# dflemin3/approxposterior

Hardware: AMD Instinct MI355X
Metric: GP-predict+acquisition candidates/sec (N_train, D fixed) (higher is better)
Workload: dtype f64

## Files before the change

### approxposterior_amd/_lib.py

```python
import ctypes
import os

_HERE = os.path.dirname(os.path.abspath(__file__))
LIB_PATH = os.path.join(_HERE, "csrc", "libapgp.so")
ABI_VERSION = 8
MAX_DIM = 32
MAX_FANTASY = 32
MAX_DRAWS = 32
MAX_FEATURES = 65536
MAX_REFS = 4096
INTEGRATED_MAX_DIM = 16

UTIL_AGP, UTIL_BAPE, UTIL_JONES, UTIL_NONE = 0, 1, 2, 3
UTIL_NEG_MEAN = 4
NM_MAX_RESTARTS = 4096
NM_MAX_FEV = 1 << 20
NM_STEPS = {1: "reflect", 2: "expand", 3: "reflect_exp", 4: "contract_out", 5: "contract_in",
            6: "shrink_out", 7: "shrink_in", 8: "maxfev"}
PRUNE_ROWS_SPLIT, PRUNE_ROWS_SIGNED = 0, 1
GMM_EM, GMM_SCORE, GMM_KMEANS = 0, 1, 2
GMM_MAX_COMP = 16
IMP_BLOCK = 256
IMP_MAX_BLOCKS = 2048

# ... 66 lines not shown
    "apgp_trsv_ex": (ctypes.c_int, [_P, _I64, _I64, _P, _F64, ctypes.c_int, _P, _P, ctypes.c_int, _P]),
    "apgp_trsv_mode": (ctypes.c_int, [ctypes.c_int]),
    "apgp_append_diag": (ctypes.c_int, [_P, _P, _F64, _P, _I64, _P]),
    "apgp_winv_apply_work_len": (_I64, [_I64]),
    "apgp_winv_apply": (ctypes.c_int, [_P, _I64, _I64, _P, _F64, ctypes.c_int, _P, _P, _P, _P]),
    "apgp_trtri_pack": (ctypes.c_int, [_P, _I64, _I64, _P, _P, _P, _P]),
    "apgp_pack_train": (ctypes.c_int, [_P, _P, _I64, _KP, _P, _P]),
    "apgp_acquire": (ctypes.c_int, [_P, _I64, _I64, _P, _P, _I64, _KP, _F64, _I32,
                                    ctypes.POINTER(_F64), ctypes.POINTER(_F64), _P,
                                    _F64, _F64, _P, _P, _P, _P, _P, _P]),
    "apgp_packed_lsolve_len": (_I64, [_I64]),
    "apgp_pack_lsolve": (ctypes.c_int, [_P, _I64, _I64, _P, _P]),
    "apgp_acquire_solve": (ctypes.c_int, [_P, _I64, _I64, _P, _P, _I64, _KP, _F64, _I32,
                                          ctypes.POINTER(_F64), ctypes.POINTER(_F64), _P,
                                          _F64, _F64, _P, _P, _P, _P, _P, _P]),
    "apgp_set_sweep_prune": (ctypes.c_int, [ctypes.c_int]),
    "apgp_get_sweep_prune": (ctypes.c_int, []),
    "apgp_set_seed_rowsplit": (ctypes.c_int, [ctypes.c_int]),
    "apgp_get_seed_rowsplit": (ctypes.c_int, []),
    "apgp_set_seed_park": (ctypes.c_int, [ctypes.c_int]),
    "apgp_get_seed_park": (ctypes.c_int, []),
    "apgp_set_prune_pipe": (ctypes.c_int, [ctypes.c_int]),
    "apgp_get_prune_pipe": (ctypes.c_int, []),
    "apgp_set_seed_first": (ctypes.c_int, [ctypes.c_int]),
    "apgp_get_seed_first": (ctypes.c_int, []),
    "apgp_set_seed_parts": (ctypes.c_int, [ctypes.c_int]),
    "apgp_get_seed_parts": (ctypes.c_int, []),
    "apgp_sweep_prune_counts_offset": (_I64, [_I64, _I64]),
    "apgp_sweep_prune_select": (ctypes.c_int, [_P, _I64, _P, _P, _F64, _P, _P]),
    "apgp_prune_bounds": (ctypes.c_int, [_P, _I64, _P, _I64, _KP, _F64, _I32, ctypes.POINTER(_F64), ctypes.POINTER(_F64),
                                         _P, _F64, _F64, ctypes.c_int, _P, _P]),
    "apgp_sweep_prune_seeds": (ctypes.c_int, [_P, _I64, _P, _P, _P]),
    "apgp_prune_rows_len": (_I64, [_I64, _I32]),
    "apgp_pack_prune_rows": (ctypes.c_int, [_P, _I64, _KP, _P, _P]),
    "apgp_acquire_rows": (ctypes.c_int, [_P, _I64, _I64, _P, _P, _I64, _KP, _F64, _I32,
                                         ctypes.POINTER(_F64), ctypes.POINTER(_F64), _P,
                                         _F64, _F64, _P, _P, _P, _P, _P, _P, _P]),
    "apgp_acquire_solve_rows": (ctypes.c_int, [_P, _I64, _I64, _P, _P, _I64, _KP, _F64, _I32,
                                               ctypes.POINTER(_F64), ctypes.POINTER(_F64), _P,
                                               _F64, _F64, _P, _P, _P, _P, _P, _P, _P]),
    "apgp_prune_bounds_rows": (ctypes.c_int, [_P, _I64, _P, _I64, _KP, _F64, _I32, ctypes.POINTER(_F64),
                                              ctypes.POINTER(_F64), _P, _F64, _F64, ctypes.c_int, _P, _P, _P]),
    "apgp_prune_srows_len": (_I64, [_I64, _I32]),
    "apgp_pack_prune_srows": (ctypes.c_int, [_P, _I64, _KP, _P, _P]),
    "apgp_acquire_rows2": (ctypes.c_int, [_P, _I64, _I64, _P, _P, _I64, _KP, _F64, _I32,
                                          ctypes.POINTER(_F64), ctypes.POINTER(_F64), _P,
# ... 108 lines not shown
```

### approxposterior_amd/csrc/sweep.hip

```cpp
#include "apgp_common.h"
#include "mma16.h"
#include "scratch.h"
#include "util_value.h"
#include <mutex>
#include <stdlib.h>
#include <string.h>

#define SW_ROWS APGP_ROW_BLOCK
#define SW_KC APGP_K_CHUNK
#define SW_TILE (SW_ROWS * SW_KC)
#define SW_CAND 64
#define SW_GRID 256
#define SW_BCH 1024
typedef unsigned int u32x4 __attribute__((ext_vector_type(4)));
#ifndef SW_KAUX
#define SW_KAUX 0
#endif

struct SweepArgs {
    const double* T;
    const double* linv;
    const double* xs;
    const unsigned char* mask;
    double* mu;
// ... 52 lines not shown
#define S2_NP (S2_ROWS / 32)
#define S2_STATIC_DIAG_NRB 8

#define S2_HQ_PRE (4 * 256)
#define S2_HQ_ACC (56 * 256)
#define S2_SPLIT_MAX 184
#define S2_PRUNE_WORDS 24
__host__ __device__ inline long long s2_fold_off(int nrb, long long ncb) {
    return (2ll * S2_SPLIT_MAX * SW_CAND * nrb + 3 * ncb + S2_PRUNE_WORDS + 1) & ~1ll;
}
__host__ __device__ inline double* s2_fold_item(double* sp_q, int nrb, long long ncb, long long pos, int jb) {
    return sp_q + s2_fold_off(nrb, ncb) + (pos * nrb + jb) * (S2_HQ_PRE + S2_HQ_ACC);
}
#define S2_HALF_COST 7
#define S2_WHOLE_COST 10
#define S2P_HALF_GEN 340
#define S2P_HALF_PARK 116
#define S2P_WHOLE_GEN 197
#define S2P_WHOLE_PARK 232
#define S2P_PAIR2_GEN 187
#define S2P_PAIR2_PARK 98
#define S2P_PAIR1_GEN 161
#define S2P_PAIR1_PARK 81
#define S2P_WAVE2 2000
#define S2W_WORD(j0, lg, p0, p1) ((2 + (j0)) | ((lg) << 8) | ((p0) << 12) | ((p1) << 20))
#define S2W_J0(sp) (((sp) & 0xff) - 2)
#define S2W_LG(sp) (((sp) >> 8) & 3)
#define S2W_P0(sp) (((sp) >> 12) & 31)
#define S2W_P1(sp) (((sp) >> 20) & 31)
#define S2W_SEED (1 << 28)
__host__ __device__ inline int s2_nkc_of(int jb, int n) {
    const int v = S2_CPB * (jb + 1), lim = (n + SW_KC - 1) / SW_KC;
    return v < lim ? v : lim;
}
__host__ __device__ inline int s2_nparts(int jb, int j0, int n, int lg) {
    if (jb < j0 || lg == 0) return 1;
    const int per = S2_ROWS >> lg, c = (n - S2_ROWS * jb + per - 1) / per;
    return c > (1 << lg) ? (1 << lg) : (c < 1 ? 1 : c);
}
__host__ __device__ inline int s2_nitems(int nrb, int j0, int n, int lg) {
    int c = 0;
    for (int jb = 0; jb < nrb; ++jb) c += s2_nparts(jb, j0, n, lg);
    return c;
}
__host__ __device__ inline int s2_part_cost(int lg) { return lg == 0 ? S2_WHOLE_COST : lg == 1 ? S2_HALF_COST : lg == 2 ? 5 : 4; }
__host__ __device__ inline void s2_row_item(int idx, int nrb, int j0, int n, int lg, int& jb, int& h) {
    int hj = nrb - 1, hh = hj >= 0 ? s2_nparts(hj, j0, n, lg) - 1 : 0, wj = (j0 < nrb ? j0 : nrb) - 1;
    const int pc = s2_part_cost(lg);
    for (int i = 0;; ++i) {
        if (hj >= j0 && (wj < 0 || pc * s2_nkc_of(hj, n) >= S2_WHOLE_COST * s2_nkc_of(wj, n))) {
            const int np = s2_nparts(hj, j0, n, lg);
            if (i == idx) { jb = hj; h = np > 1 ? hh : -1; return; }
            if (hh > 0) --hh; else { --hj; hh = hj >= 0 ? s2_nparts(hj, j0, n, lg) - 1 : 0; }
// ... 1 lines not shown
            if (i == idx || wj < 0) { jb = wj < 0 ? 0 : wj; h = -1; return; }
            --wj;
        }
    }
}
__device__ __forceinline__ double s2_q_gather(const double (&qr)[4], int lane) {
    double qs = qr[0];
#pragma unroll
    for (int r = 1; r < 4; ++r) qs += __shfl(qr[r], (lane & 48) | ((lane - 4 * r) & 15));
    qs += __shfl_xor(qs, 16);
    qs += __shfl_xor(qs, 32);
    return qs;
}
__device__ __forceinline__ bool s2_wave_skip(const SweepArgs& a, int nrb, int p0, long long pos) {
    if (p0 == 0) return false;
    const double* bmin = a.sp_q + 2ll * S2_SPLIT_MAX * SW_CAND * nrb;
    double tau = INFINITY;
    for (int i = 0; i < p0; ++i) tau = fmin(tau, a.part_u[a.blk_list[i]]);
    return !(bmin[a.blk_list[pos]] <= tau);
}

static constexpr bool s2_structured_feeder(int dpad, bool solve) { return dpad == 32 ? false : (solve ? dpad == 2 : dpad != 8); }

template <int DPAD, bool LIN, int MODE, bool LIST = false, bool RHALF = false>
__global__ __launch_bounds__(S2_THREADS, 1) void sweep2_kernel(SweepArgs a) {
    static_assert(!RHALF || (MODE == 0 && LIST), "row-half items: inverse form, list launches");
    constexpr bool SOLVE = MODE != 0;
    constexpr bool SPARK = RHALF && !LIN;
    constexpr bool STATIC_DIAG = MODE == 2;
    constexpr int XS = DPAD + 2;
    constexpr int NKK = SW_KC / 4;
    constexpr int NP = S2_NP;
    constexpr int XCHUNK16 = SW_KC * XS / 2;
    constexpr bool SF = s2_structured_feeder(DPAD, SOLVE);
    constexpr int XSTRIDE = SF ? (SW_KC * XS * 8 + 1023) / 1024 * 128 : SW_KC * XS;
    extern __shared__ __attribute__((aligned(16))) double smem[];
    double* Aring = smem;
    double* Bbuf = Aring + 3 * S2_TILE;
    double* Xbuf = Bbuf + 2 * 4 * 256;
    double* Etab = Xbuf + (SF ? 3 : 2) * XSTRIDE;
    double* Shq = Etab + APGP_EXP_TAB_N;
    double* red_u = Shq + SW_CAND;
    long long* red_i = (long long*)(red_u + 4);
    double* Cst = red_u + 8;
    const int t = threadIdx.x, lane = t & 63, w = t >> 6;
    const int cl = lane & 15, kq = lane >> 4;
    long long lst_end = 0;
    [[maybe_unused]] int wv_n = 0;
    if constexpr (LIST) {
// ... 27 lines not shown
    const int kc_lim = (a.n + SW_KC - 1) / SW_KC;
    const int nrb2 = (a.n + S2_ROWS - 1) / S2_ROWS;
    auto nkc_of = [&](int jb) { const int v = S2_CPB * (jb + 1); return v < kc_lim ? v : kc_lim; };
    auto tile_off = [&](int jb, int kc) {
        const int ib = jb >> 1;
        const unsigned tile = (unsigned)((SW_ROWS / SW_KC) * ib * (ib + 1) / 2 + kc);
        return tile * (unsigned)(SW_TILE * 8) + (unsigned)((jb & 1) * S2_TILE * 8);
    };
    int jb_lo = 0, jb_hi = nrb2;
    int rh = -1;
    long long blk0 = S2_BLK_BEGIN + blockIdx.x, blk_step = gridDim.x;
    if (a.split) {
        const int nsplit = RHALF ? wv_n : (int)(S2_BLK_END - S2_BLK_BEGIN);
        blk0 = S2_BLK_BEGIN + (int)blockIdx.x % nsplit;
        if constexpr (RHALF) {
            blk0 += S2W_P0(a.split);
            s2_row_item((int)blockIdx.x / nsplit, nrb2, S2W_J0(a.split), a.n, S2W_LG(a.split), jb_lo, rh);
        } else jb_lo = nrb2 - 1 - (int)blockIdx.x / nsplit;
        jb_hi = jb_lo + 1;
        blk_step = S2_BLK_END;
    }
    const int rpp = RHALF ? S2_NP >> S2W_LG(a.split) : S2_NP;
    const int rsh = rh > 0 ? rh * rpp : 0;
    auto successor = [&](int& jb, int& kc, long long& blk) {
        ++kc;
        if (kc >= nkc_of(jb)) { ++jb; kc = 0; }
        if (jb >= jb_hi) { jb = jb_lo; blk += blk_step; }
    };

    if (w < 4) {
        int lr[4];
#pragma unroll
        for (int r = 0; r < 4; ++r) lr[r] = (lane & 48) | ((lane + 4 * r) & 15);
        f64x2 av[2][2][2];
        auto load_a = [&](f64x2 (&dst)[2][2], int slot, int p) {
            const f64x2* A2 = (const f64x2*)(Aring + slot * S2_TILE) + lane;
#pragma unroll
            for (int h = 0; h < 2; ++h)
#pragma unroll
                for (int kp = 0; kp < 2; ++kp) dst[h][kp] = A2[((p * 2 + h) * 2 + kp) * 64];
        };
        __syncthreads();
        __syncthreads();
        __syncthreads();
        int slot = 0, bpar = 0;
        double brot[4][NKK];
        auto load_b = [&](int buf, int half) {
            const f64x2* Bw = (const f64x2*)(Bbuf + buf * 1024 + w * 256) + half * 64;
#pragma unroll
            for (int r = 0; r < 4; ++r) {
                const f64x2 bv = Bw[lr[r]];
                brot[r][2 * half] = bv.x; brot[r][2 * half + 1] = bv.y;
            }
        };
        load_a(av[0], 0, 0);
        load_b(0, 0);
        const __amdgpu_buffer_rsrc_t rs_kv = __builtin_amdgcn_make_buffer_rsrc(
            (void*)(a.kcache + (long long)blockIdx.x * a.ncache * SW_BCH), 0, (int)a.kslot_bytes, 0x00020000);
        for (long long blk = blk0; blk < S2_BLK_END; blk += blk_step) {
            double qtot = 0.0;
            for (int jb = jb_lo; jb < jb_hi; ++jb) {
                const int nkc = nkc_of(jb);
                const int ndiag0 = S2_CPB * jb;
                double qmic = 0.0;
                double acc[2 * NP][4];
#pragma unroll
                for (int s_ = 0; s_ < 2 * NP; ++s_)
#pragma unroll
                    for (int r = 0; r < 4; ++r) acc[s_][r] = 0.0;
                int kc = 0;
                auto do_tile_n = [&](auto pred_tag, auto npa_tag) {
                    constexpr bool PRED = decltype(pred_tag)::value;
                    constexpr int NPA = decltype(npa_tag)::value;
                    const int nslot = slot == 2 ? 0 : slot + 1;
                    auto mfma_pair = [&](int pr, int kk) {
#pragma unroll
                        for (int r = 0; r < 4; ++r) {
                            acc[2 * pr][r] = __builtin_amdgcn_mfma_f64_4x4x4f64(
                                av[pr & 1][0][kk >> 1][kk & 1], brot[r][kk], acc[2 * pr][r], 0, 0, 0);
                            acc[2 * pr + 1][r] = __builtin_amdgcn_mfma_f64_4x4x4f64(
                                av[pr & 1][1][kk >> 1][kk & 1], brot[r][kk], acc[2 * pr + 1][r], 0, 0, 0);
                        }
                    };
                    int p0 = (kc - ndiag0) >> 1;
                    if constexpr (RHALF) p0 -= rsh;
                    if (p0 < 0) p0 = 0;
                    int p1 = (a.n - S2_ROWS * jb + 31) >> 5;
                    if constexpr (RHALF) {
                        p1 -= rsh;
                        if (rh >= 0 && p1 > rpp) p1 = rpp;
                    }
                    if (p1 > NP) p1 = NP;
#pragma unroll
                    for (int pr = 0; pr < NPA; ++pr) {
                        const bool act = !PRED || (pr >= p0 && pr < p1);
                        if (act) mfma_pair(pr, 0);
                        __builtin_amdgcn_sched_barrier(0);
                        if (pr == NPA / 2) {
                            if constexpr (SOLVE) asm volatile("s_waitcnt vmcnt(0)" ::: "memory");
                            __syncthreads();
                        }
                        if (pr + 1 < NPA) {
                            if (pr == 0) load_b(bpar, 1);
                            load_a(av[(pr + 1) & 1], slot, pr + 1);
                            if (act) {
                                mfma_pair(pr, 1);
                                mfma_pair(pr, 2);
                                mfma_pair(pr, 3);
                            }
#if S2_SPREAD > 0
                            if (!PRED) {
#pragma unroll
                                for (int q_ = 0; q_ < (pr == 0 ? 8 : 4); ++q_) {
                                    __builtin_amdgcn_sched_group_barrier(0x100, 1, 0);
                                    __builtin_amdgcn_sched_group_barrier(0x008, S2_SPREAD, 0);
                                }
                            }
#endif
                        } else {
                            load_a(av[0], nslot, 0);
                            if (act) mfma_pair(pr, 1);
                            __builtin_amdgcn_sched_barrier(0);
                            load_b(bpar ^ 1, 0);
                            if (act) {
                                mfma_pair(pr, 2);
                                mfma_pair(pr, 3);
                            }
#if S2_SPREAD > 0
                            if (!PRED) {
#pragma unroll
                                for (int q_ = 0; q_ < 4; ++q_) {
                                    __builtin_amdgcn_sched_group_barrier(0x100, 1, 0);
                                    __builtin_amdgcn_sched_group_barrier(0x008, S2_SPREAD, 0);
                                }
                            }
#endif
                        }
                        __builtin_amdgcn_sched_barrier(0);
                    }
                    slot = nslot;
                    bpar ^= 1;
                };
                auto do_tile = [&](auto pred_tag) { do_tile_n(pred_tag, std::integral_constant<int, NP>{}); };
                if constexpr (RHALF) {
                    const int nhalf4 = (rh >= 0 && rpp == 4) ? ndiag0 : 0;
                    for (; kc < nhalf4; ++kc) do_tile_n(std::false_type{}, std::integral_constant<int, 4>{});
// ... 301 lines not shown
        const bool inb = blk < a.blk_end && crow < a.m;
        bool adm = inb, has_nan = false;
        double ktl = (LIN && a.lin_order == 0) ? (double)a.ndim : 0.0;
#pragma unroll
        for (int d = 0; d < DPAD; ++d) {
            double v = 0.0;
            if (inb && d < a.ndim) {
                v = a.T[crow * a.ndim + d];
                if (a.has_box && !(v >= Cst[APGP_MAX_DIM + d] && v <= Cst[2 * APGP_MAX_DIM + d])) adm = false;
                if (v != v) has_nan = true;
            }
            tt[d] = v * Cst[d];
            if (LIN && a.lin_order > 0) {
                const double p = v * v;
                double q = p;
                for (int e = 1; e < a.lin_order; ++e) q *= p;
                ktl += q;
            }
        }
        if (inb && a.mask && a.mask[crow] == 0) adm = false;
        fl_cur = ((adm && !has_nan) ? 1 : 0) | (has_nan ? 2 : 0) | (inb ? 4 : 0);
        ktt_cur = LIN ? fma(a.lin_coef, ktl, a.amp) : a.amp;
    };
    auto produce_b = [&](int jb, int kc, int bb, int xb) {
        double bfv[NKK];
        {
            const double* Xb = Xbuf + xb * XSTRIDE;
            double s2[NKK], s3[NKK], al[NKK], lsum[NKK];
#pragma unroll
            for (int kk = 0; kk < NKK; ++kk) {
                s2[kk] = 0.0; s3[kk] = 0.0;
                lsum[kk] = (LIN && a.lin_order == 0) ? (double)a.ndim : 0.0;
                al[kk] = Xb[(kk * 4 + kq) * XS + DPAD];
            }
#pragma unroll
            for (int d = 0; d < DPAD; d += 2)
#pragma unroll
                for (int kk = 0; kk < NKK; ++kk) {
                    const f64x2 xa = *(const f64x2*)(Xb + (kk * 4 + kq) * XS + d);
                    const double df0 = tt[d] - xa.x, df1 = tt[d + 1] - xa.y;
                    s2[kk] = fma(df0, df0, s2[kk]);
                    s3[kk] = fma(df1, df1, s3[kk]);
                    if (LIN && a.lin_order > 0) {
                        const double p0_ = tt[d] * xa.x * Cst[3 * APGP_MAX_DIM + d], p1_ = tt[d + 1] * xa.y * Cst[3 * APGP_MAX_DIM + d + 1];
                        double q0 = p0_, q1 = p1_;
                        for (int e = 1; e < a.lin_order; ++e) { q0 *= p0_; q1 *= p1_; }
                        lsum[kk] += q0 + q1;
// ... 5 lines not shown
            apgp_exp4(ex, bfv, Etab);
#pragma unroll
            for (int kk = 0; kk < NKK; ++kk) bfv[kk] = LIN ? fma(a.lin_coef, lsum[kk], bfv[kk] * a.amp) : bfv[kk] * a.amp;
            if (kc >= S2_CPB * jb) {
#pragma unroll
                for (int kk = 0; kk < NKK; ++kk) mu_cur = fma(bfv[kk], al[kk], mu_cur);
                if (kc == nkc_of(jb) - 1) {
                    double m = mu_cur;
                    m += __shfl_xor(m, 16);
                    m += __shfl_xor(m, 32);
                    mu_tot += m;
                    mu_cur = 0.0;
                }
                if (!SOLVE && !SPARK && park && jb + 1 < nrb2) {
                    const unsigned soff = (unsigned)kc * (unsigned)(SW_BCH * 8);
                    f64x2 q0, q1;
                    q0.x = bfv[0]; q0.y = bfv[1]; q1.x = bfv[2]; q1.y = bfv[3];
                    __builtin_amdgcn_raw_buffer_store_b128(__builtin_bit_cast(u32x4, q0), rs_k, hoff, soff, SW_KAUX);
                    __builtin_amdgcn_raw_buffer_store_b128(__builtin_bit_cast(u32x4, q1), rs_k, hoff, soff + 256 * 16, SW_KAUX);
                }
            }
            f64x2 o0, o1;
            o0.x = bfv[0]; o0.y = bfv[1]; o1.x = bfv[2]; o1.y = bfv[3];
            if (bb == 0) { f64x2* Bw = (f64x2*)(Bbuf + hw * 256); Bw[lane] = o0; Bw[64 + lane] = o1; }
            else { f64x2* Bw = (f64x2*)(Bbuf + 1024 + hw * 256); Bw[lane] = o0; Bw[64 + lane] = o1; }
        }
    };
    auto epilogue = [&]() {
        __syncthreads();
        if (a.split) {
            if (kq == 0) {
                const long long e = ((LIST ? blk0 : blk_fin - a.blk_begin) * SW_CAND + hw * 16 + cl) * nrb2 + jb_lo;
                if (!RHALF || rh < 0) a.sp_q[e] = Shq[hw * 16 + cl];
                if (!RHALF || rh <= 0) a.sp_mu[e] = mu_fin;
            }
            __syncthreads();
            return;
        }
        double bu = INFINITY;
        long long bi = -1;
        const long long crow = blk_fin * SW_CAND + hw * 16 + cl;
        if (kq == 0 && (fl_fin & 4)) {
            double mu = mu_fin + a.mean;
            double var = ktt_fin - Shq[hw * 16 + cl];
            if (fl_fin & 2) { mu = NAN; var = NAN; }
            if (a.mu) a.mu[crow] = mu;
            if (a.var) a.var[crow] = var;
            if (a.kind != APGP_UTIL_NONE) {
                const double uu = (fl_fin & 1) ? util_value(a.kind, mu, var, a.zeta, a.ybest) : INFINITY;
                if (a.u) a.u[crow] = uu;
                best_merge(bu, bi, uu, a.idx_offset + crow);
            }
        }
        for (int o = 8; o > 0; o >>= 1) {
            double ou = __shfl_xor(bu, o);
            long long oi = __shfl_xor(bi, o);
            best_merge(bu, bi, ou, oi);
        }
        if (lane == 0) { red_u[hw] = bu; red_i[hw] = bi; }
        __syncthreads();
        if (ht == 0 && a.kind != APGP_UTIL_NONE) {
            for (int i = 1; i < 4; ++i) best_merge(bu, bi, red_u[i], red_i[i]);
            a.part_u[blk_fin] = bu;
            a.part_i[blk_fin] = bi;
        }
    };

    if constexpr (SF) {
        const int hw_s = __builtin_amdgcn_readfirstlane(hw);
        typedef __attribute__((address_space(3))) void lds_void;
        auto dma_tile = [&](int slot, int jb, int kc) {
            double* dst = Aring + slot * S2_TILE + hw_s * 128;
            const unsigned toffs = tile_off(jb, kc);
            if constexpr (RHALF) {
                if (rh >= 0) {
#pragma unroll
                    for (int q = 0; q < 4; ++q)
                        if (q < rpp)
                            __builtin_amdgcn_raw_ptr_buffer_load_lds(rs_w, (lds_void*)(dst + q * 512), 16, (unsigned)lane * 16u,
                                                                     toffs + (unsigned)((q + rsh) * 4096) + (unsigned)hw_s * 1024u, 0, 0);
                    return;
                }
            }
#pragma unroll
            for (int q = 0; q < 8; ++q)
                __builtin_amdgcn_raw_ptr_buffer_load_lds(rs_w, (lds_void*)(dst + q * 512), 16, (unsigned)lane * 16u,
                                                         toffs + (unsigned)(q * 4096) + (unsigned)hw_s * 1024u, 0, 0);
        };
        auto dma_parked = [&](int par, int c) {
            double* dst = Bbuf + par * 1024 + hw_s * 256;
// ... 297 lines not shown
static inline long long s2_ncache(int64_t n) { return (long long)S2_CPB * (s2_nrb(n) - 1); }

template <int DPAD>
static constexpr size_t s2_lds_bytes() {
    return (3 * S2_TILE + 2 * 4 * 256 + 3 * ((SW_KC * (DPAD + 2) * 8 + 1023) / 1024 * 128) + APGP_EXP_TAB_N + SW_CAND + 8 +
            4 * APGP_MAX_DIM) * sizeof(double);
}

template <int DPAD>
static int s2_prepare_device() {
    static ApgpLdsOnce once;
    int dev = 0;
    if (hipGetDevice(&dev) != hipSuccess || dev < 0 || dev >= 64) {
        apgp_set_error("apgp_acquire: hipGetDevice failed");
        return -2;
    }
    return apgp_raise_lds(once, "apgp_acquire", dev, (int)s2_lds_bytes<DPAD>(),
                          {(const void*)sweep2_kernel<DPAD, false, 0>, (const void*)sweep2_kernel<DPAD, true, 0>,
                           (const void*)sweep2_kernel<DPAD, false, 1>, (const void*)sweep2_kernel<DPAD, true, 1>,
                           (const void*)sweep2_kernel<DPAD, false, 2>, (const void*)sweep2_kernel<DPAD, true, 2>,
                           (const void*)sweep2_kernel<DPAD, false, 0, true>, (const void*)sweep2_kernel<DPAD, true, 0, true>,
                           (const void*)sweep2_kernel<DPAD, false, 1, true>, (const void*)sweep2_kernel<DPAD, true, 1, true>,
                           (const void*)sweep2_kernel<DPAD, false, 2, true>, (const void*)sweep2_kernel<DPAD, true, 2, true>,
                           (const void*)sweep2_kernel<DPAD, false, 0, true, true>, (const void*)sweep2_kernel<DPAD, true, 0, true, true>});
}

template <int DPAD, bool LIST>
static void s2_launch(const SweepArgs& a, hipStream_t s, bool solve, unsigned grid) {
    const size_t lds = s2_lds_bytes<DPAD>();
    if (solve && a.nrb <= S2_STATIC_DIAG_NRB) {
        if (a.lin_coef != 0.0)
            hipLaunchKernelGGL((sweep2_kernel<DPAD, true, 2, LIST>), dim3(grid), dim3(S2_THREADS), lds, s, a);
        else
            hipLaunchKernelGGL((sweep2_kernel<DPAD, false, 2, LIST>), dim3(grid), dim3(S2_THREADS), lds, s, a);
    } else if (solve) {
        if (a.lin_coef != 0.0)
            hipLaunchKernelGGL((sweep2_kernel<DPAD, true, 1, LIST>), dim3(grid), dim3(S2_THREADS), lds, s, a);
        else
            hipLaunchKernelGGL((sweep2_kernel<DPAD, false, 1, LIST>), dim3(grid), dim3(S2_THREADS), lds, s, a);
    } else if (a.lin_coef != 0.0)
        hipLaunchKernelGGL((sweep2_kernel<DPAD, true, 0, LIST>), dim3(grid), dim3(S2_THREADS), lds, s, a);
    else
        hipLaunchKernelGGL((sweep2_kernel<DPAD, false, 0, LIST>), dim3(grid), dim3(S2_THREADS), lds, s, a);
}

template <int DPAD>
static int launch_sweep(const SweepArgs& a0, hipStream_t s, bool solve) {
// ... 20 lines not shown
    return 0;
}

static int g_seed_rowsplit = -1;

extern "C" int apgp_set_seed_rowsplit(int v) {
    return __atomic_exchange_n(&g_seed_rowsplit, v < 0 ? -1 : v, __ATOMIC_RELAXED);
}

extern "C" int apgp_get_seed_rowsplit(void) { return __atomic_load_n(&g_seed_rowsplit, __ATOMIC_RELAXED); }

static int g_seed_park = 1;

extern "C" int apgp_set_seed_park(int v) { return __atomic_exchange_n(&g_seed_park, v != 0 ? 1 : 0, __ATOMIC_RELAXED); }

extern "C" int apgp_get_seed_park(void) { return __atomic_load_n(&g_seed_park, __ATOMIC_RELAXED); }

static int g_prune_pipe = 1;

extern "C" int apgp_set_prune_pipe(int v) { return __atomic_exchange_n(&g_prune_pipe, v != 0 ? 1 : 0, __ATOMIC_RELAXED); }

extern "C" int apgp_get_prune_pipe(void) { return __atomic_load_n(&g_prune_pipe, __ATOMIC_RELAXED); }

#define S2_SEED_FIRST 4
static int g_seed_first = -1;

extern "C" int apgp_set_seed_first(int v) {
    return __atomic_exchange_n(&g_seed_first, v < 1 ? -1 : (v > 16 ? 16 : v), __ATOMIC_RELAXED);
}

extern "C" int apgp_get_seed_first(void) { return __atomic_load_n(&g_seed_first, __ATOMIC_RELAXED); }

static int g_seed_parts = -1;

extern "C" int apgp_set_seed_parts(int v) {
    return __atomic_exchange_n(&g_seed_parts, (v == 8 || v == 4 || v == 2 || v == 1) ? v : -1, __ATOMIC_RELAXED);
}

extern "C" int apgp_get_seed_parts(void) { return __atomic_load_n(&g_seed_parts, __ATOMIC_RELAXED); }

static long long seed_launch_cost(int nrb, int cap, int n, int j0, int lg, bool parked) {
    static const int gen[4] = {S2P_WHOLE_GEN, S2P_HALF_GEN, S2P_PAIR2_GEN, S2P_PAIR1_GEN};
    static const int park[4] = {S2P_WHOLE_PARK, S2P_HALF_PARK, S2P_PAIR2_PARK, S2P_PAIR1_PARK};
    long long load[SW_GRID] = {0};
    const int nitem = s2_nitems(nrb, j0, n, lg);
    long long last = 0;
    for (int i = 0; i < nitem; ++i) {
        int jb = 0, h = -1;
        s2_row_item(i, nrb, j0, n, lg, jb, h);
        const int kind = h >= 0 ? lg : (n - S2_ROWS * jb <= S2_ROWS / 2 ? 1 : 0);
        const int nkc = s2_nkc_of(jb, n), nre = S2_CPB * jb < nkc ? S2_CPB * jb : nkc;
        const long long c = parked ? (long long)gen[kind] * (nkc - nre) + (long long)park[kind] * nre
                                   : (long long)s2_part_cost(kind) * nkc;
        for (int k = 0; k < cap; ++k) {
            int best = 0;
            for (int q = 1; q < SW_GRID; ++q)
                if (load[q] < load[best]) best = q;
            load[best] += c;
            if (load[best] > last) last = load[best];
        }
    }
    return last;
}

struct SeedPlan { int j0, lg; long long cost; };
static SeedPlan seed_plan(int nrb, int cap, int n, bool parked) {
    const int v = apgp_get_seed_rowsplit(), fp = apgp_get_seed_parts();
    const int flg = fp == 8 ? 0 : fp == 4 ? 1 : fp == 2 ? 2 : fp == 1 ? 3 : -1;
    struct Memo { int nrb, cap, n, parked, v, flg; SeedPlan plan; };
    static std::mutex mu;
    static Memo memo[8];
    static int nmemo = 0, next = 0;
    std::lock_guard<std::mutex> g(mu);
    for (int i = 0; i < nmemo; ++i) {
        const Memo& e = memo[i];
        if (e.nrb == nrb && e.cap == cap && e.n == n && e.parked == (int)parked && e.v == v && e.flg == flg) return e.plan;
    }
    SeedPlan best = {nrb, 1, 0};
    long long best_c = -1;
    for (int lg = 1; lg <= (parked ? 2 : 1); ++lg) {
        if (flg >= 0 && lg != 1) continue;
        const int l = flg >= 0 ? flg : lg;
        for (int j0 : {nrb, nrb / 2, 0}) {
            if (v >= 0 && j0 != nrb) continue;
            const int j = v >= 0 ? (v < nrb ? v : nrb) : j0;
            if (lg > 1 && j == nrb) continue;
            const long long c = seed_launch_cost(nrb, cap, n, j, l, parked);
            if (best_c < 0 || c < best_c) { best = {j, l, c}; best_c = c; }
        }
    }
    memo[next] = {nrb, cap, n, (int)parked, v, flg, best};
    next = (next + 1) % 8;
    if (nmemo < 8) ++nmemo;
    return best;
}

template <int DPAD>
static void launch_sweep_list(const SweepArgs& a0, hipStream_t s, bool solve, const long long* list,
                              const long long* count, long long max_count, long long cap, bool rowsplit = false) {
    SweepArgs a = a0;
    const int nrb2 = s2_nrb(a.n);
    a.nrb = nrb2;
    a.blk_list = list; a.blk_count = count;
    a.blk_begin = 0; a.blk_end = (a.m + SW_CAND - 1) / SW_CAND;
    const bool can_split = !solve && nrb2 >= 2 && a.sp_q != NULL;
    if (cap > max_count) cap = max_count;
    if (can_split) {
        SweepArgs b = a;
        b.split = 1; b.ncache = 0; b.kslot_bytes = SW_BCH * 8;
        b.list_lo = 0; b.list_hi = cap;
        const bool parked = rowsplit && b.lin_coef == 0.0 && apgp_get_seed_park() != 0;
        int first = (int)cap;
        if (rowsplit && b.lin_coef == 0.0) {
            const int v = apgp_get_seed_first();
            first = v > 0 ? v : S2_SEED_FIRST;
            if (first > (int)cap) first = (int)cap;
            if (v <= 0 && first < (int)cap &&
                seed_plan(nrb2, (int)cap, b.n, true).cost - seed_plan(nrb2, first, b.n, true).cost <= S2P_WAVE2)
                first = (int)cap;
        }
        for (int wave = 0; wave < (first < (int)cap ? 2 : 1); ++wave) {
            const int p0 = wave ? first : 0, p1 = wave ? (int)cap : first, nw = p1 - p0;
            const SeedPlan plan = rowsplit ? seed_plan(nrb2, nw, b.n, parked) : SeedPlan{nrb2, 0, 0};
            const int nitem = s2_nitems(nrb2, plan.j0, b.n, plan.lg);
            b.split = S2W_WORD(plan.j0, plan.lg, p0, p1);
            if (parked) {
                b.ncache = (int)s2_ncache(b.n);
                b.kslot_bytes = (unsigned)(b.ncache * (SW_BCH * 8));
                hipLaunchKernelGGL(seed_park_kernel<DPAD>, dim3((unsigned)(nw * (b.ncache / SP_NCH))), dim3(256), 0, s, b);
            }
            if (nitem > nrb2 || parked || first < (int)cap) {
                const size_t lds = s2_lds_bytes<DPAD>();
                const unsigned grid = (unsigned)(nw * nitem);
                if (b.lin_coef != 0.0)
                    hipLaunchKernelGGL((sweep2_kernel<DPAD, true, 0, true, true>), dim3(grid), dim3(S2_THREADS), lds, s, b);
                else
                    hipLaunchKernelGGL((sweep2_kernel<DPAD, false, 0, true, true>), dim3(grid), dim3(S2_THREADS), lds, s, b);
                if (nitem > nrb2) hipLaunchKernelGGL(sweep_fold_kernel, dim3((unsigned)(nw * nrb2)), dim3(256), 0, s, b);
            } else {
                b.split = 1;
                s2_launch<DPAD, true>(b, s, solve, (unsigned)(cap * nrb2));
            }
            SweepArgs f = b;
            f.split = rowsplit ? (S2W_WORD(plan.j0, plan.lg, p0, p1) | S2W_SEED) : 1;
            hipLaunchKernelGGL(sweep_finish_kernel, dim3((unsigned)nw), dim3(64), 0, s, f);
        }
    }
    if (!can_split || max_count > cap) {
        a.split = 0;
        a.list_lo = can_split ? cap : 0; a.list_hi = APGP_MAX_M;
        s2_launch<DPAD, true>(a, s, solve, (unsigned)(max_count < SW_GRID ? max_count : SW_GRID));
    }
}

#define PR_THREADS 256
#define PR_CPT 2
#define PR_ROWS 128
#define PR_SEED 16
static inline int64_t pr_min_m(int64_t n) { return n >= 4096 ? 16384 : 65536; }
// ... 1150 lines not shown
```

### approxposterior_amd/gp.py

```python

import collections
import ctypes
import math
from operator import is_

import numpy as np
from numpy.linalg import LinAlgError
from scipy.linalg import solve_triangular

from . import _lib
from .george_extras import GeorgeExtras

__all__ = ["GP", "ExpSquaredKernel", "ConstantKernel", "Product", "ConstantModel",
           "kernels", "UTILITY_KINDS", "sobolSample"]

UTILITY_KINDS = {"agp": _lib.UTIL_AGP, "bape": _lib.UTIL_BAPE, "jones": _lib.UTIL_JONES}
SEARCH_KINDS = dict(UTILITY_KINDS, negmean=_lib.UTIL_NEG_MEAN)
NM_OPTIONS = ("adaptive", "maxiter", "maxfev", "xatol", "fatol")


def nm_coefficients(ndim, adaptive):
    if adaptive:
        dim = float(ndim)
        return 1.0, 1 + 2 / dim, 0.75 - 1 / (2 * dim), 1 - 1 / dim
# ... 353 lines not shown
        _, idx, u = self._call(t, bounds, mask, idx_offset, False)
        return idx, -u



class GP(GeorgeExtras):

    def __init__(self, kernel=None, fit_kernel=True, mean=None, fit_mean=None,
                 white_noise=None, fit_white_noise=None, solver=None, device=None,
                 **kwargs):
        if kernel is None:
            raise ValueError("a kernel is required")
        self.kernel = kernel
        self.mean = _as_model(mean, 0.0)
        self.white_noise = _as_model(white_noise, np.log(1.25e-12))
        self.fit_mean = bool(fit_mean)
        self.fit_white_noise = bool(fit_white_noise)
        self._device_arg = device
        self.variance_mode = None
        self.extend_max_rows = None
        self.sweep_prune = None
        self.seed_rowsplit = None
        self.seed_park = None
        self.seed_first = None
        self.seed_parts = None
        self.prune_signed = True
        self.prune_pipe = None
        self.sweep_prune_stats = False
        self.last_prune_counts = None
        self._computed = False
        self._x = None
        self._yerr2 = 0.0
        self._nllMemo = None
        self._rt_cache = None
        self._queries = None
        self._x_d = None
        self._mean_work = None
        self._p1_work = None
        self._imp_work = None
        self._pimp_work = None
        self._pg_work = None
        self._nll_scratch = None
        self._nll_stream = None
        self._batch = None
        self._replays = {}
        self._reset_device_state()
# ... 753 lines not shown
        ks = self._kernel_struct()
        use_solve = not self._trust_inverse()
        with self._on(torch, dev):
            st = self._stream(torch)
            if use_solve:
                self._ensure_lsolve()
            else:
                self._ensure_linv()
            self._ensure_xs(y)
            f64 = dict(dtype=torch.float64, device=dev)
            mu, var, u = (torch.empty(m, **f64) if keep else None for keep in (with_mu, with_var, with_u))
            part = torch.empty(max(int(lib.apgp_acquire_work_len(m, n)), 2), **f64)
            best = torch.empty(2, **f64)
            ev = getattr(self, "kernel_events", None)
            if ev is not None:
                e0 = torch.cuda.Event(enable_timing=True)
                e0.record()
            args = (self._xs.data_ptr(), n, ctypes.byref(ks), float(self.mean.value), kind_id, lo, hi, _ptr(mask_d),
                    float(zeta), float(np.max(y)), _ptr(mu), _ptr(var), _ptr(u), part.data_ptr(), best.data_ptr(),
                    *self._prune_stream(), st)
            prune_was = None if self.sweep_prune is None else lib.apgp_set_sweep_prune(int(self.sweep_prune))
            rowsplit_was = None if self.seed_rowsplit is None else lib.apgp_set_seed_rowsplit(int(self.seed_rowsplit))
            park_was = None if self.seed_park is None else lib.apgp_set_seed_park(int(self.seed_park))
            first_was = None if self.seed_first is None else lib.apgp_set_seed_first(int(self.seed_first))
            parts_was = None if self.seed_parts is None else lib.apgp_set_seed_parts(int(self.seed_parts))
            pipe_was = None if self.prune_pipe is None else lib.apgp_set_prune_pipe(int(self.prune_pipe))
            try:
                if use_solve:
                    _lib.check(lib.apgp_acquire_solve_rows2(T.data_ptr(), m, int(idx_offset),
                                                            self._packed_solve.data_ptr(), *args), "apgp_acquire_solve_rows2")
                else:
                    _lib.check(lib.apgp_acquire_rows2(T.data_ptr(), m, int(idx_offset), self._packed.data_ptr(), *args),
                               "apgp_acquire_rows2")
            finally:
                if prune_was is not None:
                    lib.apgp_set_sweep_prune(prune_was)
                if rowsplit_was is not None:
                    lib.apgp_set_seed_rowsplit(rowsplit_was)
                if park_was is not None:
                    lib.apgp_set_seed_park(park_was)
                if first_was is not None:
                    lib.apgp_set_seed_first(first_was)
                if parts_was is not None:
                    lib.apgp_set_seed_parts(parts_was)
                if pipe_was is not None:
                    lib.apgp_set_prune_pipe(pipe_was)
            if self.sweep_prune_stats and kind_id != _lib.UTIL_NONE and mu is None and var is None and u is None:
                off = int(lib.apgp_sweep_prune_counts_offset(m, n))
                self.last_prune_counts = part[off:off + 5].view(torch.int64).clone()
            if ev is not None:
                e1 = torch.cuda.Event(enable_timing=True)
                e1.record()
                ev.append((e0, e1))
        return _Swept(best, mu, var, u)

    def acquire(self, y, t, kind, bounds=None, mask=None, zeta=0.01, return_all=False,
                idx_offset=0, device_record=False):
        if not self.computed:
            raise RuntimeError("ERROR: Need to compute GP before using it!")
        kind_id = UTILITY_KINDS[str(kind).lower()]
        if device_record and return_all:
            raise ValueError("device_record returns the arg-min record only")
        torch, dev, _ = self._rt()
# ... 980 lines not shown
```

### include/apgp.h

```cpp
#ifndef APGP_H
#define APGP_H

#include <stddef.h>
#include <stdint.h>

#ifdef __cplusplus
extern "C" {
#endif

#define APGP_ABI_VERSION 8
#define APGP_MAX_DIM 32
#define APGP_ROW_BLOCK 512
#define APGP_K_CHUNK 16
#define APGP_CAND_BLOCK 64

#define APGP_UTIL_AGP 0
#define APGP_UTIL_BAPE 1
#define APGP_UTIL_JONES 2
#define APGP_UTIL_NONE 3
#define APGP_UTIL_NEG_MEAN 4

typedef struct apgp_kernel {
    int32_t ndim;
    int32_t lin_order;
// ... 65 lines not shown

int apgp_pack_train(const double* X, const double* alpha, int64_t n,
                    const apgp_kernel_t* kern , double* xs, void* stream);

int64_t apgp_acquire_work_len(int64_t m, int64_t n);
int apgp_acquire(const double* T, int64_t m, int64_t idx_offset,
                 const double* packed_linv, const double* xs, int64_t n,
                 const apgp_kernel_t* kern , double mean, int32_t kind,
                 const double* lo , const double* hi ,
                 const uint8_t* mask, double zeta, double ybest,
                 double* mu, double* var, double* u,
                 void* part, apgp_best_t* best, void* stream);

int64_t apgp_packed_lsolve_len(int64_t n);
int apgp_pack_lsolve(const double* L, int64_t n, int64_t ldl, double* packed, void* stream);
int apgp_acquire_solve(const double* T, int64_t m, int64_t idx_offset,
                       const double* packed_lsolve, const double* xs, int64_t n,
                       const apgp_kernel_t* kern , double mean, int32_t kind,
                       const double* lo , const double* hi ,
                       const uint8_t* mask, double zeta, double ybest,
                       double* mu, double* var, double* u,
                       void* part, apgp_best_t* best, void* stream);

int apgp_set_sweep_prune(int v);
int apgp_get_sweep_prune(void);
int apgp_set_seed_rowsplit(int v);
int apgp_get_seed_rowsplit(void);
int apgp_set_seed_park(int v);
int apgp_get_seed_park(void);
int apgp_set_prune_pipe(int v);
int apgp_get_prune_pipe(void);
int apgp_set_seed_first(int v);
int apgp_get_seed_first(void);
int apgp_set_seed_parts(int v);
int apgp_get_seed_parts(void);
int64_t apgp_sweep_prune_counts_offset(int64_t m, int64_t n);
int apgp_sweep_prune_select(const double* bmin, int64_t ncb, const int64_t* seeds, int64_t* counts,
                            double tau, int64_t* list, void* stream);
int apgp_prune_bounds(const double* T, int64_t m, const double* xs, int64_t n,
                      const apgp_kernel_t* kern , double mean, int32_t kind,
                      const double* lo , const double* hi , const uint8_t* mask,
                      double zeta, double ybest, int coarse, double* bmin_out, void* stream);
int apgp_sweep_prune_seeds(const double* bmin, int64_t ncb, int64_t* seeds, int64_t* counts, void* stream);

int64_t apgp_prune_rows_len(int64_t n, int32_t ndim);
int apgp_pack_prune_rows(const double* xs, int64_t n, const apgp_kernel_t* kern , void* rows, void* stream);
// ... 250 lines not shown
```

Baseline: 976.0 million.

## Add deep LDS stage ring with DMA prefetch for parked seed sweep items

```diff
diff --git a/approxposterior_amd/_lib.py b/approxposterior_amd/_lib.py
--- a/approxposterior_amd/_lib.py
+++ b/approxposterior_amd/_lib.py
@@ -112,6 +112,8 @@
     "apgp_get_seed_park": (ctypes.c_int, []),
     "apgp_set_prune_pipe": (ctypes.c_int, [ctypes.c_int]),
     "apgp_get_prune_pipe": (ctypes.c_int, []),
+    "apgp_set_seed_prefetch": (ctypes.c_int, [ctypes.c_int]),
+    "apgp_get_seed_prefetch": (ctypes.c_int, []),
     "apgp_set_seed_first": (ctypes.c_int, [ctypes.c_int]),
     "apgp_get_seed_first": (ctypes.c_int, []),
     "apgp_set_seed_parts": (ctypes.c_int, [ctypes.c_int]),
diff --git a/approxposterior_amd/csrc/sweep.hip b/approxposterior_amd/csrc/sweep.hip
--- a/approxposterior_amd/csrc/sweep.hip
+++ b/approxposterior_amd/csrc/sweep.hip
@@ -98,6 +98,12 @@
 #define S2P_PAIR2_PARK 98
 #define S2P_PAIR1_GEN 161
 #define S2P_PAIR1_PARK 81
+#define S2Q_HALF_GEN 220
+#define S2Q_HALF_PARK 101
+#define S2Q_PAIR2_GEN 183
+#define S2Q_PAIR2_PARK 54
+#define S2Q_PAIR1_GEN 183
+#define S2Q_PAIR1_PARK 45
 #define S2P_WAVE2 2000
 #define S2W_WORD(j0, lg, p0, p1) ((2 + (j0)) | ((lg) << 8) | ((p0) << 12) | ((p1) << 20))
 #define S2W_J0(sp) (((sp) & 0xff) - 2)
@@ -105,6 +111,13 @@
 #define S2W_P0(sp) (((sp) >> 12) & 31)
 #define S2W_P1(sp) (((sp) >> 20) & 31)
 #define S2W_SEED (1 << 28)
+#define S2W_PF(sp) (((sp) >> 25) & 7)
+#define S2_STAGE(pp) ((pp) * 512 + 2 * 4 * 128)
+#define S2_NRING(pp) (3 * S2_TILE / S2_STAGE(pp))
+static_assert(S2_NRING(4) == 4 && S2_NRING(2) == 6 && S2_NRING(1) == 8, "the stage ring fits the three tile slots");
+static_assert(S2_NRING(4) * S2_STAGE(4) <= 3 * S2_TILE && S2_NRING(2) * S2_STAGE(2) <= 3 * S2_TILE &&
+              S2_NRING(1) * S2_STAGE(1) <= 3 * S2_TILE, "the stage ring fits the three tile slots");
+static_assert(S2_NRING(4) - 3 == 1 && S2_NRING(2) - 3 == 3 && S2_NRING(1) - 3 == 5, "the DEEP loop's vmcnt cases follow the ring");
 __host__ __device__ inline int s2_nkc_of(int jb, int n) {
     const int v = S2_CPB * (jb + 1), lim = (n + SW_KC - 1) / SW_KC;
     return v < lim ? v : lim;
@@ -152,9 +165,10 @@
 
 static constexpr bool s2_structured_feeder(int dpad, bool solve) { return dpad == 32 ? false : (solve ? dpad == 2 : dpad != 8); }
 
-template <int DPAD, bool LIN, int MODE, bool LIST = false, bool RHALF = false>
+template <int DPAD, bool LIN, int MODE, bool LIST = false, bool RHALF = false, bool DEEP = false>
 __global__ __launch_bounds__(S2_THREADS, 1) void sweep2_kernel(SweepArgs a) {
     static_assert(!RHALF || (MODE == 0 && LIST), "row-half items: inverse form, list launches");
+    static_assert(!DEEP || (RHALF && !LIN), "stage ring: the parked seed route");
     constexpr bool SOLVE = MODE != 0;
     constexpr bool SPARK = RHALF && !LIN;
     constexpr bool STATIC_DIAG = MODE == 2;
@@ -228,6 +242,9 @@
     }
     const int rpp = RHALF ? S2_NP >> S2W_LG(a.split) : S2_NP;
     const int rsh = rh > 0 ? rh * rpp : 0;
+    [[maybe_unused]] const bool deep = DEEP && rh >= 0 && a.ncache > 0;
+    [[maybe_unused]] const int sstr = deep ? S2_STAGE(rpp) : S2_TILE;
+    [[maybe_unused]] const int nring = deep ? (rpp == 4 ? S2_NRING(4) : rpp == 2 ? S2_NRING(2) : S2_NRING(1)) : 3;
     auto successor = [&](int& jb, int& kc, long long& blk) {
         ++kc;
         if (kc >= nkc_of(jb)) { ++jb; kc = 0; }
@@ -240,7 +257,7 @@
         for (int r = 0; r < 4; ++r) lr[r] = (lane & 48) | ((lane + 4 * r) & 15);
         f64x2 av[2][2][2];
         auto load_a = [&](f64x2 (&dst)[2][2], int slot, int p) {
-            const f64x2* A2 = (const f64x2*)(Aring + slot * S2_TILE) + lane;
+            const f64x2* A2 = (const f64x2*)(Aring + slot * (DEEP ? sstr : S2_TILE)) + lane;
 #pragma unroll
             for (int h = 0; h < 2; ++h)
 #pragma unroll
@@ -251,8 +268,9 @@
         __syncthreads();
         int slot = 0, bpar = 0;
         double brot[4][NKK];
-        auto load_b = [&](int buf, int half) {
+        auto load_b = [&](int buf, int half, [[maybe_unused]] int stg = 0) {
             const f64x2* Bw = (const f64x2*)(Bbuf + buf * 1024 + w * 256) + half * 64;
+            if constexpr (DEEP) { if (deep) Bw = (const f64x2*)(Aring + stg * sstr + rpp * 512 + w * 256) + half * 64; }
 #pragma unroll
             for (int r = 0; r < 4; ++r) {
                 const f64x2 bv = Bw[lr[r]];
@@ -278,7 +296,7 @@
                 auto do_tile_n = [&](auto pred_tag, auto npa_tag) {
                     constexpr bool PRED = decltype(pred_tag)::value;
                     constexpr int NPA = decltype(npa_tag)::value;
-                    const int nslot = slot == 2 ? 0 : slot + 1;
+                    const int nslot = slot == (DEEP ? nring - 1 : 2) ? 0 : slot + 1;
                     auto mfma_pair = [&](int pr, int kk) {
 #pragma unroll
                         for (int r = 0; r < 4; ++r) {
@@ -307,7 +325,7 @@
                             __syncthreads();
                         }
                         if (pr + 1 < NPA) {
-                            if (pr == 0) load_b(bpar, 1);
+                            if (pr == 0) load_b(bpar, 1, slot);
                             load_a(av[(pr + 1) & 1], slot, pr + 1);
                             if (act) {
                                 mfma_pair(pr, 1);
@@ -327,7 +345,7 @@
                             load_a(av[0], nslot, 0);
                             if (act) mfma_pair(pr, 1);
                             __builtin_amdgcn_sched_barrier(0);
-                            load_b(bpar ^ 1, 0);
+                            load_b(bpar ^ 1, 0, nslot);
                             if (act) {
                                 mfma_pair(pr, 2);
                                 mfma_pair(pr, 3);
@@ -675,7 +693,7 @@
         fl_cur = ((adm && !has_nan) ? 1 : 0) | (has_nan ? 2 : 0) | (inb ? 4 : 0);
         ktt_cur = LIN ? fma(a.lin_coef, ktl, a.amp) : a.amp;
     };
-    auto produce_b = [&](int jb, int kc, int bb, int xb) {
+    auto produce_b = [&](int jb, int kc, int bb, int xb, [[maybe_unused]] int stg = -1) {
         double bfv[NKK];
         {
             const double* Xb = Xbuf + xb * XSTRIDE;
@@ -727,6 +745,9 @@
             }
             f64x2 o0, o1;
             o0.x = bfv[0]; o0.y = bfv[1]; o1.x = bfv[2]; o1.y = bfv[3];
+            if constexpr (DEEP) {
+                if (stg >= 0) { f64x2* Bw = (f64x2*)(Aring + stg * sstr + rpp * 512 + hw * 256); Bw[lane] = o0; Bw[64 + lane] = o1; return; }
+            }
             if (bb == 0) { f64x2* Bw = (f64x2*)(Bbuf + hw * 256); Bw[lane] = o0; Bw[64 + lane] = o1; }
             else { f64x2* Bw = (f64x2*)(Bbuf + 1024 + hw * 256); Bw[lane] = o0; Bw[64 + lane] = o1; }
         }
@@ -771,6 +792,85 @@
         }
     };
 
+    if constexpr (DEEP) {
+        if (deep) {
+            const int hw_s = __builtin_amdgcn_readfirstlane(hw);
+            typedef __attribute__((address_space(3))) void lds_void;
+            const int jb = jb_lo, nt = nkc_of(jb);
+            const int nd0 = S2_CPB * jb < nt ? S2_CPB * jb : nt;
+            int dist = S2W_PF(a.split);
+            dist = dist < 1 ? 1 : (dist > nring - 2 ? nring - 2 : dist);
+            const int nreq = rpp + 2;
+            auto dma_stage = [&](int stg, int kc) {
+                double* dst = Aring + stg * sstr + hw_s * 128;
+                const unsigned toffs = tile_off(jb, kc);
+#pragma unroll
+                for (int q = 0; q < 4; ++q)
+                    if (q < rpp)
+                        __builtin_amdgcn_raw_ptr_buffer_load_lds(rs_w, (lds_void*)(dst + q * 512), 16, (unsigned)lane * 16u,
+                                                                 toffs + (unsigned)((q + rsh) * 4096) + (unsigned)hw_s * 1024u, 0, 0);
+            };
+            auto dma_stage_b = [&](int stg, int c) {
+                double* dst = Aring + stg * sstr + rpp * 512 + hw_s * 256;
+                const unsigned soff = (unsigned)c * (unsigned)(SW_BCH * 8) + (unsigned)hw_s * 1024u;
+                __builtin_amdgcn_raw_ptr_buffer_load_lds(rs_k, (lds_void*)dst, 16, (unsigned)lane * 16u, soff, 0, SW_KAUX);
+                __builtin_amdgcn_raw_ptr_buffer_load_lds(rs_k, (lds_void*)(dst + 128), 16, (unsigned)lane * 16u, soff + 4096u, 0, SW_KAUX);
+            };
+            const int g1 = nd0 > 1 ? nd0 : 1;
+            __syncthreads();
+            load_candidates(blk0);
+            dma_stage(0, 0);
+            x_put(0, x_fetch(0));
+            x_put(1, x_fetch(g1 < nt ? g1 : 0));
+            __syncthreads();
+            produce_b(jb, 0, 0, 0, 0);
+            XQ xq = x_fetch(g1 + 1 < nt ? g1 + 1 : 0);
+            __syncthreads();
+            int nx = 1, stx = 1;
+            int st1 = 1, g = 1;
+            for (int i = 0; i < nt; ++i) {
+                const int t1 = i + 1;
+                int n_pend = 0;
+                if (t1 >= nd0) {
+                    if (t1 < nt) {
+                        __builtin_amdgcn_s_setprio(3);
+                        dma_stage(st1, t1);
+                        produce_b(jb, t1, 0, g & 1, st1);
+                        x_put((g & 1) ^ 1, xq);
+                        if (t1 + 2 < nt) { xq = x_fetch(t1 + 2); n_pend = X2 ? 2 : 1; }
+                        ++g;
+                        __builtin_amdgcn_s_setprio(0);
+                    }
+                } else {
+                    while (nx < nd0 && nx <= i + dist) {
+                        dma_stage(stx, nx);
+                        dma_stage_b(stx, nx);
+                        ++nx;
+                        stx = stx + 1 == nring ? 0 : stx + 1;
+                    }
+                    n_pend = (nx - 1 - t1) * nreq;
+                }
+                st1 = st1 + 1 == nring ? 0 : st1 + 1;
+#define S2_DEEP_BARRIER(n) asm volatile("s_waitcnt vmcnt(" #n ") lgkmcnt(0)\n\ts_barrier" ::: "memory")
+                switch (n_pend) {
+                    case 1: S2_DEEP_BARRIER(1); break;
+                    case 2: S2_DEEP_BARRIER(2); break;
+                    case 3: S2_DEEP_BARRIER(3); break;
+                    case 4: S2_DEEP_BARRIER(4); break;
+                    case 6: S2_DEEP_BARRIER(6); break;
+                    case 8: S2_DEEP_BARRIER(8); break;
+                    case 9: S2_DEEP_BARRIER(9); break;
+                    case 12: S2_DEEP_BARRIER(12); break;
+                    case 15: S2_DEEP_BARRIER(15); break;
+                    default: S2_DEEP_BARRIER(0); break;
+                }
+#undef S2_DEEP_BARRIER
+            }
+            load_candidates(S2_BLK_END);
+            epilogue();
+            return;
+        }
+    }
     if constexpr (SF) {
         const int hw_s = __builtin_amdgcn_readfirstlane(hw);
         typedef __attribute__((address_space(3))) void lds_void;
@@ -1114,7 +1214,8 @@
                            (const void*)sweep2_kernel<DPAD, false, 0, true>, (const void*)sweep2_kernel<DPAD, true, 0, true>,
                            (const void*)sweep2_kernel<DPAD, false, 1, true>, (const void*)sweep2_kernel<DPAD, true, 1, true>,
                            (const void*)sweep2_kernel<DPAD, false, 2, true>, (const void*)sweep2_kernel<DPAD, true, 2, true>,
-                           (const void*)sweep2_kernel<DPAD, false, 0, true, true>, (const void*)sweep2_kernel<DPAD, true, 0, true, true>});
+                           (const void*)sweep2_kernel<DPAD, false, 0, true, true>, (const void*)sweep2_kernel<DPAD, true, 0, true, true>,
+                           (const void*)sweep2_kernel<DPAD, false, 0, true, true, true>});
 }
 
 template <int DPAD, bool LIST>
@@ -1181,6 +1282,16 @@
 
 extern "C" int apgp_get_prune_pipe(void) { return __atomic_load_n(&g_prune_pipe, __ATOMIC_RELAXED); }
 
+#define S2_PREFETCH_MAX 6
+static_assert(S2_PREFETCH_MAX == S2_NRING(1) - 2 && S2_PREFETCH_MAX <= 7, "the deepest ring's distance, in three bits of split");
+static int g_seed_prefetch = S2_PREFETCH_MAX;
+
+extern "C" int apgp_set_seed_prefetch(int v) {
+    return __atomic_exchange_n(&g_seed_prefetch, v < 0 ? 0 : (v > S2_PREFETCH_MAX ? S2_PREFETCH_MAX : v), __ATOMIC_RELAXED);
+}
+
+extern "C" int apgp_get_seed_prefetch(void) { return __atomic_load_n(&g_seed_prefetch, __ATOMIC_RELAXED); }
+
 #define S2_SEED_FIRST 4
 static int g_seed_first = -1;
 
@@ -1198,9 +1309,13 @@
 
 extern "C" int apgp_get_seed_parts(void) { return __atomic_load_n(&g_seed_parts, __ATOMIC_RELAXED); }
 
-static long long seed_launch_cost(int nrb, int cap, int n, int j0, int lg, bool parked) {
+enum { S2R_PLAIN = 0, S2R_PARKED = 1, S2R_RING = 2 };
+static long long seed_launch_cost(int nrb, int cap, int n, int j0, int lg, int route) {
     static const int gen[4] = {S2P_WHOLE_GEN, S2P_HALF_GEN, S2P_PAIR2_GEN, S2P_PAIR1_GEN};
     static const int park[4] = {S2P_WHOLE_PARK, S2P_HALF_PARK, S2P_PAIR2_PARK, S2P_PAIR1_PARK};
+    static const int gen_ring[4] = {S2P_WHOLE_GEN, S2Q_HALF_GEN, S2Q_PAIR2_GEN, S2Q_PAIR1_GEN};
+    static const int park_ring[4] = {S2P_WHOLE_PARK, S2Q_HALF_PARK, S2Q_PAIR2_PARK, S2Q_PAIR1_PARK};
+    const bool parked = route != S2R_PLAIN;
     long long load[SW_GRID] = {0};
     const int nitem = s2_nitems(nrb, j0, n, lg);
     long long last = 0;
@@ -1209,7 +1324,8 @@
         s2_row_item(i, nrb, j0, n, lg, jb, h);
         const int kind = h >= 0 ? lg : (n - S2_ROWS * jb <= S2_ROWS / 2 ? 1 : 0);
         const int nkc = s2_nkc_of(jb, n), nre = S2_CPB * jb < nkc ? S2_CPB * jb : nkc;
-        const long long c = parked ? (long long)gen[kind] * (nkc - nre) + (long long)park[kind] * nre
+        const bool ring = route == S2R_RING && h >= 0;
+        const long long c = parked ? (long long)(ring ? gen_ring : gen)[kind] * (nkc - nre) + (long long)(ring ? park_ring : park)[kind] * nre
                                    : (long long)s2_part_cost(kind) * nkc;
         for (int k = 0; k < cap; ++k) {
             int best = 0;
@@ -1223,32 +1339,32 @@
 }
 
 struct SeedPlan { int j0, lg; long long cost; };
-static SeedPlan seed_plan(int nrb, int cap, int n, bool parked) {
+static SeedPlan seed_plan(int nrb, int cap, int n, int route) {
     const int v = apgp_get_seed_rowsplit(), fp = apgp_get_seed_parts();
     const int flg = fp == 8 ? 0 : fp == 4 ? 1 : fp == 2 ? 2 : fp == 1 ? 3 : -1;
-    struct Memo { int nrb, cap, n, parked, v, flg; SeedPlan plan; };
+    struct Memo { int nrb, cap, n, route, v, flg; SeedPlan plan; };
     static std::mutex mu;
     static Memo memo[8];
     static int nmemo = 0, next = 0;
     std::lock_guard<std::mutex> g(mu);
     for (int i = 0; i < nmemo; ++i) {
         const Memo& e = memo[i];
-        if (e.nrb == nrb && e.cap == cap && e.n == n && e.parked == (int)parked && e.v == v && e.flg == flg) return e.plan;
+        if (e.nrb == nrb && e.cap == cap && e.n == n && e.route == route && e.v == v && e.flg == flg) return e.plan;
     }
     SeedPlan best = {nrb, 1, 0};
     long long best_c = -1;
-    for (int lg = 1; lg <= (parked ? 2 : 1); ++lg) {
+    for (int lg = 1; lg <= (route == S2R_RING ? 3 : route == S2R_PARKED ? 2 : 1); ++lg) {
         if (flg >= 0 && lg != 1) continue;
         const int l = flg >= 0 ? flg : lg;
         for (int j0 : {nrb, nrb / 2, 0}) {
             if (v >= 0 && j0 != nrb) continue;
             const int j = v >= 0 ? (v < nrb ? v : nrb) : j0;
             if (lg > 1 && j == nrb) continue;
-            const long long c = seed_launch_cost(nrb, cap, n, j, l, parked);
+            const long long c = seed_launch_cost(nrb, cap, n, j, l, route);
             if (best_c < 0 || c < best_c) { best = {j, l, c}; best_c = c; }
         }
     }
-    memo[next] = {nrb, cap, n, (int)parked, v, flg, best};
+    memo[next] = {nrb, cap, n, route, v, flg, best};
     next = (next + 1) % 8;
     if (nmemo < 8) ++nmemo;
     return best;
@@ -1269,18 +1385,19 @@
         b.split = 1; b.ncache = 0; b.kslot_bytes = SW_BCH * 8;
         b.list_lo = 0; b.list_hi = cap;
         const bool parked = rowsplit && b.lin_coef == 0.0 && apgp_get_seed_park() != 0;
+        const int kroute = apgp_get_seed_prefetch() > 0 ? S2R_RING : S2R_PARKED;
         int first = (int)cap;
         if (rowsplit && b.lin_coef == 0.0) {
             const int v = apgp_get_seed_first();
             first = v > 0 ? v : S2_SEED_FIRST;
             if (first > (int)cap) first = (int)cap;
             if (v <= 0 && first < (int)cap &&
-                seed_plan(nrb2, (int)cap, b.n, true).cost - seed_plan(nrb2, first, b.n, true).cost <= S2P_WAVE2)
+                seed_plan(nrb2, (int)cap, b.n, kroute).cost - seed_plan(nrb2, first, b.n, kroute).cost <= S2P_WAVE2)
                 first = (int)cap;
         }
         for (int wave = 0; wave < (first < (int)cap ? 2 : 1); ++wave) {
             const int p0 = wave ? first : 0, p1 = wave ? (int)cap : first, nw = p1 - p0;
-            const SeedPlan plan = rowsplit ? seed_plan(nrb2, nw, b.n, parked) : SeedPlan{nrb2, 0, 0};
+            const SeedPlan plan = rowsplit ? seed_plan(nrb2, nw, b.n, parked ? kroute : S2R_PLAIN) : SeedPlan{nrb2, 0, 0};
             const int nitem = s2_nitems(nrb2, plan.j0, b.n, plan.lg);
             b.split = S2W_WORD(plan.j0, plan.lg, p0, p1);
             if (parked) {
@@ -1291,9 +1408,14 @@
             if (nitem > nrb2 || parked || first < (int)cap) {
                 const size_t lds = s2_lds_bytes<DPAD>();
                 const unsigned grid = (unsigned)(nw * nitem);
+                const int pf = parked ? apgp_get_seed_prefetch() : 0;
                 if (b.lin_coef != 0.0)
                     hipLaunchKernelGGL((sweep2_kernel<DPAD, true, 0, true, true>), dim3(grid), dim3(S2_THREADS), lds, s, b);
-                else
+                else if (pf > 0) {
+                    SweepArgs d = b;
+                    d.split |= pf << 25;
+                    hipLaunchKernelGGL((sweep2_kernel<DPAD, false, 0, true, true, true>), dim3(grid), dim3(S2_THREADS), lds, s, d);
+                } else
                     hipLaunchKernelGGL((sweep2_kernel<DPAD, false, 0, true, true>), dim3(grid), dim3(S2_THREADS), lds, s, b);
                 if (nitem > nrb2) hipLaunchKernelGGL(sweep_fold_kernel, dim3((unsigned)(nw * nrb2)), dim3(256), 0, s, b);
             } else {
diff --git a/approxposterior_amd/gp.py b/approxposterior_amd/gp.py
--- a/approxposterior_amd/gp.py
+++ b/approxposterior_amd/gp.py
@@ -399,6 +399,7 @@
         self.sweep_prune = None
         self.seed_rowsplit = None
         self.seed_park = None
+        self.seed_prefetch = None
         self.seed_first = None
         self.seed_parts = None
         self.prune_signed = True
@@ -1198,6 +1199,7 @@
             prune_was = None if self.sweep_prune is None else lib.apgp_set_sweep_prune(int(self.sweep_prune))
             rowsplit_was = None if self.seed_rowsplit is None else lib.apgp_set_seed_rowsplit(int(self.seed_rowsplit))
             park_was = None if self.seed_park is None else lib.apgp_set_seed_park(int(self.seed_park))
+            prefetch_was = None if self.seed_prefetch is None else lib.apgp_set_seed_prefetch(int(self.seed_prefetch))
             first_was = None if self.seed_first is None else lib.apgp_set_seed_first(int(self.seed_first))
             parts_was = None if self.seed_parts is None else lib.apgp_set_seed_parts(int(self.seed_parts))
             pipe_was = None if self.prune_pipe is None else lib.apgp_set_prune_pipe(int(self.prune_pipe))
@@ -1215,6 +1217,8 @@
                     lib.apgp_set_seed_rowsplit(rowsplit_was)
                 if park_was is not None:
                     lib.apgp_set_seed_park(park_was)
+                if prefetch_was is not None:
+                    lib.apgp_set_seed_prefetch(prefetch_was)
                 if first_was is not None:
                     lib.apgp_set_seed_first(first_was)
                 if parts_was is not None:
diff --git a/include/apgp.h b/include/apgp.h
--- a/include/apgp.h
+++ b/include/apgp.h
@@ -111,6 +111,8 @@
                        double* mu, double* var, double* u,
                        void* part, apgp_best_t* best, void* stream);
 
+int apgp_set_seed_prefetch(int v);
+int apgp_get_seed_prefetch(void);
 int apgp_set_sweep_prune(int v);
 int apgp_get_sweep_prune(void);
 int apgp_set_seed_rowsplit(int v);
```

New measurement: 1.065 billion (median of 6 runs). 1.09x the previous value.
